# sjz5202/DisenLink

Measured on AMD Instinct MI355X. Metric: edges/sec (aggregate+score) at K=8 d=64, higher is better.
Workload: dtype f32; 1 GPU; squirrel_real (edge list of the parity fixture)(seed 0): N=5201, edge rows=217073, 85/5/10 split, E_sym=342129, scored train pairs P=1009603 (m=5), K=8, d=64, beta=0.5, t=1.0; forward route+aggregate+score_pairs; K=8, d=64, n_nodes=5201, E_sym=342129, P=1009603

## Files before the change

disenlink_amd/csrc/dl_score.hip:

```cpp
#include "dl_fast.h"
#include "dl_score_bwd.h"

namespace dl {
namespace fast {

template <int K, int D, typename T, bool COEF>
__global__ __launch_bounds__(BLOCK, K <= 8 ? 4 : 1) void score_fwd_seg_kernel(dl_csr_plan g, const int32_t* __restrict__ pair_id,
                                                              const int32_t* __restrict__ pair_id2,
                                                              const T* __restrict__ Z, const T* __restrict__ H,
                                                              float t, float* __restrict__ prob,
                                                              float* __restrict__ coef_e,
                                                              float* __restrict__ coef_q) {
    using GE = Geo<K, D, T>;
    constexpr int VEC = GE::VEC, G = GE::G, EPW = GE::EPW, ROW = GE::ROW;
    constexpr int KB = K > 8 ? 8 : K;
    using FLB = FactorLanes<G, KB>;
    constexpr int KBP = FLB::KP;
    __shared__ __attribute__((aligned(16))) float urow[WAVES_PER_BLOCK][2 * ROW];
    const WaveSeg ws = load_wave_seg(g);
    const SegInfo si = ws.si;
    const int wave = ws.wave, lane = lane_id();
    const bool active = ws.active;
    if (active) stage_u_rows<K, D, T>(urow[wave], Z, H, (size_t)si.grow);
    __syncthreads();
    if (!active) return;
    const int c = lane % G, grp = lane / G;
    const int kbb = FLB::factor_base(c);
    int my_col = si.grow, my_pair = 0, my_pair2 = -1;
    if (si.beg + lane < si.end) {
        my_col = g.col[si.beg + lane];
        my_pair = pair_id[si.beg + lane];
        if (pair_id2 != nullptr) my_pair2 = pair_id2[si.beg + lane];
    }
    for (int base = si.beg; base < si.end; base += EPW) {
        const int it = base + grp;
        const bool live = it < si.end;
        const size_t v = (size_t)entry_scalar<EPW>(my_col, base - si.beg, grp);
        const int q = entry_scalar<EPW>(my_pair, base - si.beg, grp);
        const int q2 = entry_scalar<EPW>(my_pair2, base - si.beg, grp);
        float term = 0.0f;
#pragma unroll
        for (int b0 = 0; b0 < K; b0 += KB) {
            float pq[KBP], ps[KBP];
#pragma unroll
            for (int k = 0; k < KBP; ++k) {
                const bool in = k < KB && b0 + k < K;
                const int kk = in ? b0 + k : 0;
                pq[k] = in ? dot(load_f32<VEC>(&urow[wave][ROW + kk * D + c * VEC]), Tab<T>::load(H + v * ROW + kk * D + c * VEC)) : 0.0f;
                ps[k] = in ? dot(load_f32<VEC>(&urow[wave][kk * D + c * VEC]), Tab<T>::load(Z + v * ROW + kk * D + c * VEC)) : 0.0f;
            }
            TransposedReduce<KBP, G / 2>::run(pq, c);
            TransposedReduce<KBP, G / 2>::run(ps, c);
#pragma unroll
            for (int i = 0; i < FLB::VPL; ++i) {
                const int k = b0 + kbb + i;
                if (FLB::primary(c) && kbb + i < KB && k < K) {
                    const float ek = expf(div_t(ps[i], t));
                    const float qe = pq[i] * ek;
                    term += qe;
                    if (COEF && live) {
                        coef_e[(size_t)q * K + k] = ek;
                        coef_q[(size_t)q * K + k] = qe;
                        if (q2 >= 0) {
                            coef_e[(size_t)q2 * K + k] = ek;
                            coef_q[(size_t)q2 * K + k] = qe;
                        }
                    }
                }
            }
        }
        const float logit = group_allreduce_sum<G>(term);
        if (live && c == 0) {
            const float p = sigmoid_ref(logit);
            prob[q] = p;
            if (q2 >= 0) prob[q2] = p;
        }
    }
}

constexpr int FWD_WAVE_MAXW = 6;
template <int K, int D>
struct FwdWave {
    static constexpr bool ok = D == 64 && (K == 4 || K == 8);
    static constexpr int NJ = K * D / 256, U = 4;
};

template <int K, int D, bool T1, bool COEF, bool FOLD>
__global__ __launch_bounds__(BLOCK) __attribute__((amdgpu_waves_per_eu(4, FWD_WAVE_MAXW))) void score_fwd_wave_kernel(dl_csr_plan g, const int32_t* __restrict__ pair_id,
                                                                  const int32_t* __restrict__ pair_id2,
                                                                  const float* __restrict__ Z, const float* __restrict__ H, float t,
                                                                  float* __restrict__ prob, float* __restrict__ coef_e,
                                                                  float* __restrict__ coef_q) {
    using FW = FwdWave<K, D>;
    constexpr int NJ = FW::NJ, U = FW::U, ROW = K * D;
    static_assert(D == 64 && NJ >= 1 && U * NJ <= 8, "one DPP row of 16 lanes per factor slice; at most 8 exponents per row and step");
    __shared__ __attribute__((aligned(16))) float4 urow[WAVES_PER_BLOCK][2 * ROW / 4];
    __shared__ int ent_q[WAVES_PER_BLOCK][(FOLD ? 2 : 1) * DL_WAVE];
    const WaveSeg ws = load_wave_seg(g);
    if (!ws.active) return;
    const SegInfo si = ws.si;
    const int wave = ws.wave, lane = lane_id();
    const int i = lane & 15, r = lane >> 4;
    float4* const mine = urow[wave];
#pragma unroll
    for (int j = 0; j < NJ; ++j) {
        mine[j * 64 + lane] = *reinterpret_cast<const float4*>(Z + (size_t)si.grow * ROW + (j * 64 + lane) * 4);
        mine[ROW / 4 + j * 64 + lane] = *reinterpret_cast<const float4*>(H + (size_t)si.grow * ROW + (j * 64 + lane) * 4);
    }
    int my_col = si.grow, my_q = 0, my_q2 = -1;
    if (si.beg + lane < si.end) {
        my_col = g.col[si.beg + lane];
        my_q = pair_id[si.beg + lane];
        if constexpr (FOLD) my_q2 = pair_id2[si.beg + lane];
    }
    ent_q[wave][lane] = my_q;
    if constexpr (FOLD) ent_q[wave][DL_WAVE + lane] = my_q2;
    const int len = si.end - si.beg;
    auto do_step = [&](const int step, auto tail, const int n_live) {
        constexpr bool TAIL = decltype(tail)::value;
        float4 zv[U][NJ], hv[U][NJ];
#pragma unroll
        for (int e = 0; e < U; ++e) {
            if (!TAIL || e < n_live) {
                const size_t v = (size_t)(unsigned)__builtin_amdgcn_readlane(my_col, (step * U + e) & 63);
                const auto* zr = uniform_row<dl_vf4>(Z, v * ROW * sizeof(float));
                const auto* hr = uniform_row<dl_vf4>(H, v * ROW * sizeof(float));
#pragma unroll
                for (int j = 0; j < NJ; ++j) {
                    zv[e][j] = as_float4(zr[(unsigned)(lane + j * 64)]);
                    hv[e][j] = as_float4(hr[(unsigned)(lane + j * 64)]);
                }
            } else {
#pragma unroll
                for (int j = 0; j < NJ; ++j) zv[e][j] = hv[e][j] = make_float4(0.0f, 0.0f, 0.0f, 0.0f);
            }
        }
        float val[16];
#pragma unroll
        for (int x = 0; x < 16; ++x) val[x] = 0.0f;
#pragma unroll
        for (int j = 0; j < NJ; ++j) {
            const float4 a4 = mine[j * 64 + lane], b4 = mine[ROW / 4 + j * 64 + lane];
#pragma unroll
            for (int e = 0; e < U; ++e) {
                val[j * 4 + e] = dot4_packed(a4, zv[e][j]);
                val[8 + j * 4 + e] = dot4_packed(b4, hv[e][j]);
            }
            __builtin_amdgcn_sched_barrier(0);
        }
        TransposedReduce<16, 8>::run(val, i);
        const float mine_v = val[0];
        const float ex = expf(T1 ? mine_v : mine_v / t);
        const float ttv = mine_v * xor_lane<8>(ex);
        float term = ttv;
        if constexpr (NJ == 2) term += xor_lane<4>(ttv);
        const float logit = add_xor<32>(add_xor<16>(term));
        const float p = sigmoid_ref(logit);
        const int idx = step * U + (i & 3);
        const bool live = idx < len;
        const int qq = ent_q[wave][idx & 63];
        int qq2 = -1;
        if constexpr (FOLD) qq2 = ent_q[wave][DL_WAVE + (idx & 63)];
        if (lane >= 8 && lane < 12 && live) {
            prob[qq] = p;
            if (FOLD && qq2 >= 0) prob[qq2] = p;
        }
        if constexpr (COEF) {
            const int k = 4 * ((i & 7) >> 2) + r;
            if (live && (NJ == 2 || (i & 7) < 4)) {
                if (i < 8) coef_e[(size_t)qq * K + k] = ex;
                else coef_q[(size_t)qq * K + k] = ttv;
                if (FOLD && qq2 >= 0) {
                    if (i < 8) coef_e[(size_t)qq2 * K + k] = ex;
                    else coef_q[(size_t)qq2 * K + k] = ttv;
                }
            }
        }
    };
    const int nfull = len / U;
    for (int step = 0; step < nfull; ++step) do_step(step, std::false_type{}, U);
    if (len % U != 0) do_step(nfull, std::true_type{}, len % U);
}

namespace hub {
constexpr int WAVES = 8, THREADS = WAVES * DL_WAVE;

typedef int dl_vi4 __attribute__((ext_vector_type(4)));
__device__ __forceinline__ dl_vi4 plan_words(const int32_t* a, int idx) {
    const auto* g = (const __attribute__((address_space(1))) int32_t*)a;
    return reinterpret_cast<const __attribute__((address_space(4))) dl_vi4*>((const __attribute__((address_space(4))) int32_t*)g)[idx];
}

struct StepWords {
    dl_vi4 v, u, q, p;
};

template <int K, int D, bool T1, bool COEF, bool FOLD>
__global__ __launch_bounds__(THREADS) __attribute__((amdgpu_waves_per_eu(4, 4))) void score_fwd_wave_kernel(
    dl_pair_hub h, const float* __restrict__ Z, const float* __restrict__ H, float t, float* __restrict__ prob,
    float* __restrict__ coef_e, float* __restrict__ coef_q) {
    using FW = FwdWave<K, D>;
    constexpr int NJ = FW::NJ, U = FW::U, ROW = K * D, R4 = 2 * ROW / 4;
    static_assert(D == 64 && NJ >= 1 && U == 4 && U * NJ <= 8, "the step geometry of score_fwd_wave_kernel");
    static_assert(DL_HUB_W == 2 * WAVES, "every wave stages two rows of the block");
    __shared__ __attribute__((aligned(16))) float4 urow[DL_HUB_W * R4];
    const int x = blockIdx.x % h.n_slices;
    const int it = h.slice_item0[x] + (int)(blockIdx.x / h.n_slices);
    if (it >= h.slice_item0[x + 1]) return;
    const int wave = wave_index(), lane = lane_id();
    const int i = lane & 15, r = lane >> 4;
    const int blk = h.item_block[it];
    const int s_a = h.item_step[4 * it], s_b = h.item_step[4 * it + 1], s_c = h.item_step[4 * it + 2],
              s_end = h.item_step[4 * it + 3];
#pragma unroll
    for (int rr = 0; rr < 2; ++rr) {
        const int ul = 2 * wave + rr;
        const int row = h.block_row[blk * DL_HUB_W + ul];
#pragma unroll
        for (int j = 0; j < NJ; ++j) {
            float4 a = make_float4(0.0f, 0.0f, 0.0f, 0.0f), b = a;
            if (row >= 0) {
                a = *reinterpret_cast<const float4*>(Z + (size_t)row * ROW + (j * 64 + lane) * 4);
                b = *reinterpret_cast<const float4*>(H + (size_t)row * ROW + (j * 64 + lane) * 4);
            }
            urow[ul * R4 + j * 64 + lane] = a;
            urow[ul * R4 + ROW / 4 + j * 64 + lane] = b;
        }
    }
    __syncthreads();
    auto fetch = [&](const int step) {
        const int s = __builtin_amdgcn_readfirstlane(step);
        StepWords w;
        w.v = plan_words(h.step_v, s), w.u = plan_words(h.step_u, s), w.q = plan_words(h.step_q, s);
        w.p = dl_vi4{-1, -1, -1, -1};
        if constexpr (FOLD) w.p = plan_words(h.step_q2, s);
        return w;
    };
    auto do_step = [&](const StepWords& w, auto shape, auto last) {
        constexpr int NV = decltype(shape)::value;
        constexpr bool LAST = decltype(last)::value;
        const int sv[4] = {w.v.x, w.v.y, w.v.z, w.v.w}, su[4] = {w.u.x, w.u.y, w.u.z, w.u.w}, sq[4] = {w.q.x, w.q.y, w.q.z, w.q.w},
                  sq2[4] = {w.p.x, w.p.y, w.p.z, w.p.w};
        float4 zv[NV][NJ], hv[NV][NJ];
#pragma unroll
        for (int n = 0; n < NV; ++n) {
            if (!LAST || sv[n] >= 0) {
                const size_t v = (size_t)(unsigned)sv[n];
                const auto* zr = uniform_row<dl_vf4>(Z, v * ROW * sizeof(float));
                const auto* hr = uniform_row<dl_vf4>(H, v * ROW * sizeof(float));
#pragma unroll
                for (int j = 0; j < NJ; ++j) {
                    zv[n][j] = as_float4(zr[(unsigned)(lane + j * 64)]);
                    hv[n][j] = as_float4(hr[(unsigned)(lane + j * 64)]);
                }
            } else {
#pragma unroll
                for (int j = 0; j < NJ; ++j) zv[n][j] = hv[n][j] = make_float4(0.0f, 0.0f, 0.0f, 0.0f);
            }
        }
        float val[16];
#pragma unroll
        for (int q = 0; q < 16; ++q) val[q] = 0.0f;
#pragma unroll
        for (int j = 0; j < NJ; ++j) {
            float4 a4[U], b4[U];
#pragma unroll
            for (int e = 0; e < U; ++e) {
                const float4* mine = urow + (su[e] & (DL_HUB_W - 1)) * R4;
                a4[e] = mine[j * 64 + lane], b4[e] = mine[ROW / 4 + j * 64 + lane];
            }
            __builtin_amdgcn_sched_barrier(0);
#pragma unroll
            for (int e = 0; e < U; ++e) {
                val[j * 4 + e] = dot4_packed(a4[e], zv[e * NV / 4][j]);
                val[8 + j * 4 + e] = dot4_packed(b4[e], hv[e * NV / 4][j]);
            }
            __builtin_amdgcn_sched_barrier(0);
        }
        TransposedReduce<16, 8>::run(val, i);
        const float mine_v = val[0];
        const float ex = expf(T1 ? mine_v : mine_v / t);
        const float ttv = mine_v * xor_lane<8>(ex);
        float term = ttv;
        if constexpr (NJ == 2) term += xor_lane<4>(ttv);
        const float logit = add_xor<32>(add_xor<16>(term));
        const float p = sigmoid_ref(logit);
        const int e_me = i & 3;
        const int qq = e_me == 0 ? sq[0] : e_me == 1 ? sq[1] : e_me == 2 ? sq[2] : sq[3];
        const int qq2 = e_me == 0 ? sq2[0] : e_me == 1 ? sq2[1] : e_me == 2 ? sq2[2] : sq2[3];
        const bool live = qq >= 0;
        if (lane >= 8 && lane < 12 && live) {
            prob[qq] = p;
            if (FOLD && qq2 >= 0) prob[qq2] = p;
        }
        if constexpr (COEF) {
            const int k = 4 * ((i & 7) >> 2) + r;
            if (live && (NJ == 2 || (i & 7) < 4)) {
                if (i < 8) coef_e[(size_t)qq * K + k] = ex;
                else coef_q[(size_t)qq * K + k] = ttv;
                if (FOLD && qq2 >= 0) {
                    if (i < 8) coef_e[(size_t)qq2 * K + k] = ex;
                    else coef_q[(size_t)qq2 * K + k] = ttv;
                }
            }
        }
    };
    using FULL = std::false_type;
    using LAST = std::true_type;
    constexpr std::integral_constant<int, 4> SHAPE_A{};
    constexpr std::integral_constant<int, 2> SHAPE_B{};
    constexpr std::integral_constant<int, 1> SHAPE_C{};
    int s = s_a + wave;
    StepWords nxt = {};
    if (s < s_end) nxt = fetch(s);
    auto take = [&](const int step) {
        const StepWords w = nxt;
        if (step + WAVES < s_end) nxt = fetch(step + WAVES);
        return w;
    };
    for (; s < s_b - 1; s += WAVES) do_step(take(s), SHAPE_A, FULL{});
    if (s == s_b - 1) do_step(take(s), SHAPE_A, LAST{}), s += WAVES;
    for (; s < s_c - 1; s += WAVES) do_step(take(s), SHAPE_B, FULL{});
    if (s == s_c - 1) do_step(take(s), SHAPE_B, LAST{}), s += WAVES;
    for (; s < s_end; s += WAVES) do_step(take(s), SHAPE_C, FULL{});
}
}

template <int K, int D, typename T>
__global__ __launch_bounds__(BLOCK) void score_allpairs_kernel(const T* __restrict__ Z, const T* __restrict__ H, int N,
                                                               float t, int n_slices, int slice_w, int chunks_per_u,
                                                               float* __restrict__ prob) {
    using GE = Geo<K, D, T>;
    constexpr int VEC = GE::VEC, G = GE::G, EPW = GE::EPW, ROW = GE::ROW;
    constexpr int KB = K > 8 ? 8 : K;
    using FLB = FactorLanes<G, KB>;
    constexpr int KBP = FLB::KP;
    constexpr int VCH = 256;
    __shared__ __attribute__((aligned(16))) float urow[WAVES_PER_BLOCK][2 * ROW];
    const int wave = threadIdx.x >> 6, lane = lane_id();
    const int x = blockIdx.x % n_slices;
    const int item = (blockIdx.x / n_slices) * WAVES_PER_BLOCK + wave;
    const int u = item / chunks_per_u, ch = item - u * chunks_per_u;
    const int v0 = x * slice_w + ch * VCH;
    const int v1 = min(min(v0 + VCH, (x + 1) * slice_w), N);
    const bool active = u < N && v0 < v1;
    if (active) stage_u_rows<K, D, T>(urow[wave], Z, H, (size_t)u);
    __syncthreads();
    if (!active) return;
    const int c = lane % G, grp = lane / G;
    const int kbb = FLB::factor_base(c);
    for (int base = v0; base < v1; base += EPW) {
        const int vi = base + grp;
        const bool live = vi < v1;
        const size_t v = (size_t)(live ? vi : v0);
        float term = 0.0f;
#pragma unroll
        for (int b0 = 0; b0 < K; b0 += KB) {
            float pq[KBP], ps[KBP];
#pragma unroll
            for (int k = 0; k < KBP; ++k) {
                const bool in = k < KB && b0 + k < K;
                const int kk = in ? b0 + k : 0;
                pq[k] = in ? dot(load_f32<VEC>(&urow[wave][ROW + kk * D + c * VEC]), Tab<T>::load(H + v * ROW + kk * D + c * VEC)) : 0.0f;
                ps[k] = in ? dot(load_f32<VEC>(&urow[wave][kk * D + c * VEC]), Tab<T>::load(Z + v * ROW + kk * D + c * VEC)) : 0.0f;
            }
            TransposedReduce<KBP, G / 2>::run(pq, c);
            TransposedReduce<KBP, G / 2>::run(ps, c);
#pragma unroll
            for (int i = 0; i < FLB::VPL; ++i)
                if (FLB::primary(c) && kbb + i < KB && b0 + kbb + i < K) term += pq[i] * expf(div_t(ps[i], t));
        }
        const float logit = group_allreduce_sum<G>(term);
        if (live && c == 0) prob[(size_t)u * N + vi] = sigmoid_ref(logit);
    }
}

template <int K, int D, typename T, int PASS>
__global__ __launch_bounds__(BLOCK) void score_bwd_coef_seg_kernel(dl_csr_plan g, const int32_t* __restrict__ inc_pair,
                                                                   const T* __restrict__ X, float t,
                                                                   const float* __restrict__ prob,
                                                                   const float* __restrict__ g_prob,
                                                                   const float* __restrict__ coef,
                                                                   float* __restrict__ out, float* __restrict__ part) {
    using GE = Geo<K, D, T>;
    constexpr int VEC = GE::VEC, G = GE::G, EPW = GE::EPW, ROW = GE::ROW;
    using US = Stage<K, D, T, 1>;
    __shared__ __attribute__((aligned(16))) float red[US::FLOATS];
    const WaveSeg ws = load_wave_seg(g);
    const SegInfo si = ws.si;
    const int lane = lane_id();
    const int c = lane % G, grp = lane / G;
    if (ws.active) {
        Chunk<VEC> acc[K];
#pragma unroll
        for (int k = 0; k < K; ++k) acc[k] = zero_chunk<VEC>();
        int my_col = si.grow, my_pair = 0;
        float my_gl = 0.0f;
        if (si.beg + lane < si.end) {
            my_col = g.col[si.beg + lane];
            my_pair = inc_pair[si.beg + lane];
            const float pr = prob[my_pair];
            my_gl = g_prob[my_pair] * pr * (1.0f - pr);
            if (PASS == 0) my_gl = div_t(my_gl, t);
        }
        for (int base = si.beg; base < si.end; base += EPW) {
            const int idx = base + grp - si.beg;
            const size_t v = (size_t)__shfl(my_col, idx, DL_WAVE);
            const int q = __shfl(my_pair, idx, DL_WAVE);
            const float gl = __shfl(my_gl, idx, DL_WAVE);
            float ck[K];
            if constexpr (K % 4 == 0) {
#pragma unroll
                for (int k = 0; k < K; k += 4) {
                    const float4 t4 = *reinterpret_cast<const float4*>(coef + (size_t)q * K + k);
                    ck[k] = t4.x; ck[k + 1] = t4.y; ck[k + 2] = t4.z; ck[k + 3] = t4.w;
                }
            } else {
#pragma unroll
                for (int k = 0; k < K; ++k) ck[k] = coef[(size_t)q * K + k];
            }
#pragma unroll
            for (int b0 = 0; b0 < K; b0 += 8) {
                Chunk<VEC> xv[8];
#pragma unroll
                for (int k = 0; k < 8; ++k)
                    if (b0 + k < K) xv[k] = Tab<T>::load(X + v * ROW + (b0 + k) * D + c * VEC);
#pragma unroll
                for (int k = 0; k < 8; ++k)
                    if (b0 + k < K) fma_chunk(acc[b0 + k], gl * ck[b0 + k], xv[k]);
            }
        }
        US::put(red, ws.wave, grp, c, acc, 0);
    }
    __syncthreads();
    if (!ws.head) return;
    float4 r[US::NQ];
    US::sum(red, ws.wave, ws.n_unit, lane, r);
    float* o = si.slot < 0 ? out + (size_t)si.grow * ROW : part + (size_t)si.slot * ROW;
#pragma unroll
    for (int q = 0; q < US::NQ; ++q) {
        const int x = q * DL_WAVE + lane;
        if (x < US::F4) store4(o + 4 * x, r[q]);
    }
}

struct AllpairsGeo { int n_slices, slice_w, chunks_per_u; long long items; unsigned blocks; };
static AllpairsGeo allpairs_geo(int N, size_t row_bytes) {
    AllpairsGeo g;
    const double table = 2.0 * N * (double)row_bytes;
    g.n_slices = table <= 8.0 * 8.0 * (4 << 20) && N >= 64 ? 8 : 1;
    g.slice_w = (N + g.n_slices - 1) / g.n_slices;
    g.chunks_per_u = (g.slice_w + 255) / 256;
    g.items = (long long)N * g.chunks_per_u;
    g.blocks = (unsigned)(g.n_slices * ((g.items + WAVES_PER_BLOCK - 1) / WAVES_PER_BLOCK));
    return g;
}

template <int K, int D, typename T>
struct ScoreOps {
    static constexpr int ROW = K * D;
    static int score_fwd(const dl_pair_incidence* by_u, const void* Z, const void* H, float t, float* prob,
                         float* coef, hipStream_t st) {
        const dl_csr_plan* g = &by_u->csr;
        float* coef_q = coef ? coef + (size_t)by_u->n_pairs * K : nullptr;
        if constexpr (std::is_same<T, float>::value && FwdWave<K, D>::ok) {
            if (g->seg_len <= 64 && g->seg_len % FwdWave<K, D>::U == 0 && !config().fwd_group_kernel) {
                auto pick = [&](auto launch) {
                    auto fold = [&](auto t1, auto cf) {
                        if (by_u->inc_pair2) launch(t1, cf, std::true_type{});
                        else launch(t1, cf, std::false_type{});
                    };
                    if (coef) { if (t == 1.0f) fold(std::true_type{}, std::true_type{}); else fold(std::false_type{}, std::true_type{}); }
                    else { if (t == 1.0f) fold(std::true_type{}, std::false_type{}); else fold(std::false_type{}, std::false_type{}); }
                };
                auto wave_plan = [&](const dl_csr_plan* c, const int32_t* pair, const int32_t* pair2) {
                    pick([&](auto t1, auto cf, auto fo) {
                        hipLaunchKernelGGL((score_fwd_wave_kernel<K, D, decltype(t1)::value, decltype(cf)::value, decltype(fo)::value>),
                                           dim3(seg_blocks(c)), dim3(BLOCK), 0, st, *c, pair, pair2, (const float*)Z,
                                           (const float*)H, t, prob, coef, coef_q);
                    });
                };
                const dl_pair_hub* hp = config().fwd_hub ? by_u->hub : nullptr;
                if (hp != nullptr && hp->n_items > 0) {
                    pick([&](auto t1, auto cf, auto fo) {
                        hipLaunchKernelGGL((hub::score_fwd_wave_kernel<K, D, decltype(t1)::value, decltype(cf)::value, decltype(fo)::value>),
                                           dim3((unsigned)hp->n_slices * (unsigned)hp->slice_max_item), dim3(hub::THREADS), 0,
                                           st, *hp, (const float*)Z, (const float*)H, t, prob, coef, coef_q);
                    });
                    if (hp->rest.n_entries > 0) wave_plan(&hp->rest, hp->rest_pair, hp->rest_pair2);
                    return check_launch("score_pairs_fwd(fast, hub blocks + wave per entry)");
                }
                wave_plan(g, by_u->inc_pair, by_u->inc_pair2);
                return check_launch("score_pairs_fwd(fast, wave per entry)");
            }
        }
        if (coef)
            hipLaunchKernelGGL((score_fwd_seg_kernel<K, D, T, true>), dim3(seg_blocks(g)), dim3(BLOCK), 0, st, *g,
                               by_u->inc_pair, by_u->inc_pair2, (const T*)Z, (const T*)H, t, prob, coef, coef_q);
        else
            hipLaunchKernelGGL((score_fwd_seg_kernel<K, D, T, false>), dim3(seg_blocks(g)), dim3(BLOCK), 0, st, *g,
                               by_u->inc_pair, by_u->inc_pair2, (const T*)Z, (const T*)H, t, prob, coef, coef_q);
        return check_launch("score_pairs_fwd(fast)");
    }

    static int score_allpairs(const void* Z, const void* H, int N, float t, float* prob, hipStream_t st) {
        const AllpairsGeo g = allpairs_geo(N, ROW * sizeof(T));
        hipLaunchKernelGGL((score_allpairs_kernel<K, D, T>), dim3(g.blocks), dim3(BLOCK), 0, st, (const T*)Z, (const T*)H, N,
                           t, g.n_slices, g.slice_w, g.chunks_per_u, prob);
        return check_launch("score_allpairs_fwd(fast)");
    }

    static int score_bwd(const dl_pair_incidence* inc, const void* Z, const void* H, float t, const float* prob,
                         const float* g_prob, const float* coef, float* dZ, float* dH, float* part, hipStream_t st) {
        const dl_csr_plan* g = &inc->csr;
        const float* no_x = nullptr;
        if (coef) {
            const float* coef_q = coef + (size_t)inc->n_pairs * K;
            float* part_h = part + (size_t)g->n_slots * ROW;
            hipLaunchKernelGGL((score_bwd_coef_seg_kernel<K, D, T, 0>), dim3(seg_blocks(g)), dim3(BLOCK), 0, st, *g,
                               inc->inc_pair, (const T*)Z, t, prob, g_prob, coef_q, dZ, part);
            hipLaunchKernelGGL((score_bwd_coef_seg_kernel<K, D, T, 1>), dim3(seg_blocks(g)), dim3(BLOCK), 0, st, *g,
                               inc->inc_pair, (const T*)H, t, prob, g_prob, coef, dH, part_h);
            if (g->n_multi > 0)
                hipLaunchKernelGGL((row_combine_kernel<ROW, float, float>), dim3(g->n_multi, 2), dim3(BLOCK), 0, st, *g,
                                   part, ROW, no_x, 0.0f, 1.0f, dZ, 0, part_h, dH);
            return check_launch("score_pairs_bwd(fast, stored terms)");
        }
        hipLaunchKernelGGL((score_bwd_seg_kernel<K, D, T, false>), dim3(seg_blocks(g)), dim3(BLOCK), 0, st, *g, inc->inc_pair,
                           (const T*)Z, (const T*)H, t, prob, g_prob, dZ, dH, part);
        if (g->n_multi > 0)
            hipLaunchKernelGGL((row_combine_kernel<ROW, float, float>), dim3(g->n_multi, 2), dim3(BLOCK), 0, st, *g, part,
                               2 * ROW, no_x, 0.0f, 1.0f, dZ, 0, part + ROW, dH);
        return check_launch("score_pairs_bwd(fast)");
    }
};

}

int fast_score_pairs_fwd(const dl_pair_incidence* by_u, const void* Z, const void* H, int K, int d, int dtype,
                         float t, float* prob, float* coef, hipStream_t st) {
#define X_F32(KK, DD) if (K == KK && d == DD) return fast::ScoreOps<KK, DD, float>::score_fwd(by_u, Z, H, t, prob, coef, st);
#define X_BF16(KK, DD) if (K == KK && d == DD) return fast::ScoreOps<KK, DD, fast::bf16_t>::score_fwd(by_u, Z, H, t, prob, coef, st);
    DL_DISPATCH(X)
#undef X_F32
#undef X_BF16
}

int fast_score_pairs_bwd(const dl_pair_incidence* inc, const void* Z, const void* H, int K, int d, int dtype,
                         float t, const float* prob, const float* g_prob, const float* coef, float* dZ, float* dH,
                         float* part, hipStream_t st) {
#define X_F32(KK, DD) if (K == KK && d == DD) return fast::ScoreOps<KK, DD, float>::score_bwd(inc, Z, H, t, prob, g_prob, coef, dZ, dH, part, st);
#define X_BF16(KK, DD) if (K == KK && d == DD) return fast::ScoreOps<KK, DD, fast::bf16_t>::score_bwd(inc, Z, H, t, prob, g_prob, coef, dZ, dH, part, st);
    DL_DISPATCH(X)
#undef X_F32
#undef X_BF16
}

int fast_score_allpairs_fwd(const void* Z, const void* H, int N, int K, int d, int dtype, float t, float* prob,
                            hipStream_t st) {
#define X_F32(KK, DD) if (K == KK && d == DD) return fast::ScoreOps<KK, DD, float>::score_allpairs(Z, H, N, t, prob, st);
#define X_BF16(KK, DD) if (K == KK && d == DD) return fast::ScoreOps<KK, DD, fast::bf16_t>::score_allpairs(Z, H, N, t, prob, st);
    DL_DISPATCH(X)
#undef X_F32
#undef X_BF16
}

void fast_score_allpairs_form(int N, int K, int d, int dtype, int* out) {
    const fast::AllpairsGeo g = fast::allpairs_geo(N, (size_t)K * d * (dtype == DL_BF16 ? sizeof(fast::bf16_t) : sizeof(float)));
    out[1] = (int)g.items;
    out[2] = (int)g.blocks;
    out[3] = g.n_slices;
    out[4] = g.slice_w;
    out[5] = g.chunks_per_u;
}

}
```

Baseline: 8.341 billion edges/s.

## Batch pair logits across steps and use masked DPP transposed reduction

In the score wave kernel without coefficient output, each wave now collects one logit per step into a per-lane slot over 16 steps. Every 16 steps it runs sigmoid once and each of the 64 lanes writes its own probability, replacing the per-step sigmoid and 4-lane scattered store. Pair-index loads move into a per-batch gather instead of per-step scalar plan loads. The 16-wide transposed reduction is replaced with inline DPP asm using bank masks to cut instructions. The cost is more complex lane bookkeeping and hand-written asm hazards (s_nop) that could be fragile.

```diff
diff --git a/disenlink_amd/csrc/dl_score.hip b/disenlink_amd/csrc/dl_score.hip
--- a/disenlink_amd/csrc/dl_score.hip
+++ b/disenlink_amd/csrc/dl_score.hip
@@ -195,6 +195,45 @@
     dl_vi4 v, u, q, p;
 };
 
+__device__ __forceinline__ void transposed_reduce16_masked(float* v, int c) {
+    float a[8], b[4];
+    asm volatile("s_nop 1\n\t"
+                 "v_add_f32_dpp %0, %8, %8 row_ror:8 row_mask:0xf bank_mask:0x3\n\t"
+                 "v_add_f32_dpp %1, %9, %9 row_ror:8 row_mask:0xf bank_mask:0x3\n\t"
+                 "v_add_f32_dpp %2, %10, %10 row_ror:8 row_mask:0xf bank_mask:0x3\n\t"
+                 "v_add_f32_dpp %3, %11, %11 row_ror:8 row_mask:0xf bank_mask:0x3\n\t"
+                 "v_add_f32_dpp %4, %12, %12 row_ror:8 row_mask:0xf bank_mask:0x3\n\t"
+                 "v_add_f32_dpp %5, %13, %13 row_ror:8 row_mask:0xf bank_mask:0x3\n\t"
+                 "v_add_f32_dpp %6, %14, %14 row_ror:8 row_mask:0xf bank_mask:0x3\n\t"
+                 "v_add_f32_dpp %7, %15, %15 row_ror:8 row_mask:0xf bank_mask:0x3\n\t"
+                 "v_add_f32_dpp %0, %16, %16 row_ror:8 row_mask:0xf bank_mask:0xc\n\t"
+                 "v_add_f32_dpp %1, %17, %17 row_ror:8 row_mask:0xf bank_mask:0xc\n\t"
+                 "v_add_f32_dpp %2, %18, %18 row_ror:8 row_mask:0xf bank_mask:0xc\n\t"
+                 "v_add_f32_dpp %3, %19, %19 row_ror:8 row_mask:0xf bank_mask:0xc\n\t"
+                 "v_add_f32_dpp %4, %20, %20 row_ror:8 row_mask:0xf bank_mask:0xc\n\t"
+                 "v_add_f32_dpp %5, %21, %21 row_ror:8 row_mask:0xf bank_mask:0xc\n\t"
+                 "v_add_f32_dpp %6, %22, %22 row_ror:8 row_mask:0xf bank_mask:0xc\n\t"
+                 "v_add_f32_dpp %7, %23, %23 row_ror:8 row_mask:0xf bank_mask:0xc"
+                 : "=&v"(a[0]), "=&v"(a[1]), "=&v"(a[2]), "=&v"(a[3]), "=&v"(a[4]), "=&v"(a[5]), "=&v"(a[6]), "=&v"(a[7])
+                 : "v"(v[0]), "v"(v[1]), "v"(v[2]), "v"(v[3]), "v"(v[4]), "v"(v[5]), "v"(v[6]), "v"(v[7]), "v"(v[8]), "v"(v[9]),
+                   "v"(v[10]), "v"(v[11]), "v"(v[12]), "v"(v[13]), "v"(v[14]), "v"(v[15]));
+    asm volatile("s_nop 1\n\t"
+                 "v_add_f32_dpp %0, %4, %4 row_shl:4 row_mask:0xf bank_mask:0x5\n\t"
+                 "v_add_f32_dpp %1, %5, %5 row_shl:4 row_mask:0xf bank_mask:0x5\n\t"
+                 "v_add_f32_dpp %2, %6, %6 row_shl:4 row_mask:0xf bank_mask:0x5\n\t"
+                 "v_add_f32_dpp %3, %7, %7 row_shl:4 row_mask:0xf bank_mask:0x5\n\t"
+                 "v_add_f32_dpp %0, %8, %8 row_shr:4 row_mask:0xf bank_mask:0xa\n\t"
+                 "v_add_f32_dpp %1, %9, %9 row_shr:4 row_mask:0xf bank_mask:0xa\n\t"
+                 "v_add_f32_dpp %2, %10, %10 row_shr:4 row_mask:0xf bank_mask:0xa\n\t"
+                 "v_add_f32_dpp %3, %11, %11 row_shr:4 row_mask:0xf bank_mask:0xa\n\t"
+                 "s_nop 1"
+                 : "=&v"(b[0]), "=&v"(b[1]), "=&v"(b[2]), "=&v"(b[3])
+                 : "v"(a[0]), "v"(a[1]), "v"(a[2]), "v"(a[3]), "v"(a[4]), "v"(a[5]), "v"(a[6]), "v"(a[7]));
+#pragma unroll
+    for (int q = 0; q < 4; ++q) v[q] = b[q];
+    TransposedReduce<4, 2>::run(v, c);
+}
+
 template <int K, int D, bool T1, bool COEF, bool FOLD>
 __global__ __launch_bounds__(THREADS) __attribute__((amdgpu_waves_per_eu(4, 4))) void score_fwd_wave_kernel(
     dl_pair_hub h, const float* __restrict__ Z, const float* __restrict__ H, float t, float* __restrict__ prob,
@@ -203,6 +242,7 @@
     constexpr int NJ = FW::NJ, U = FW::U, ROW = K * D, R4 = 2 * ROW / 4;
     static_assert(D == 64 && NJ >= 1 && U == 4 && U * NJ <= 8, "the step geometry of score_fwd_wave_kernel");
     static_assert(DL_HUB_W == 2 * WAVES, "every wave stages two rows of the block");
+    constexpr bool BATCH = !COEF;
     __shared__ __attribute__((aligned(16))) float4 urow[DL_HUB_W * R4];
     const int x = blockIdx.x % h.n_slices;
     const int it = h.slice_item0[x] + (int)(blockIdx.x / h.n_slices);
@@ -231,10 +271,38 @@
     auto fetch = [&](const int step) {
         const int s = __builtin_amdgcn_readfirstlane(step);
         StepWords w;
-        w.v = plan_words(h.step_v, s), w.u = plan_words(h.step_u, s), w.q = plan_words(h.step_q, s);
-        w.p = dl_vi4{-1, -1, -1, -1};
-        if constexpr (FOLD) w.p = plan_words(h.step_q2, s);
+        w.v = plan_words(h.step_v, s), w.u = plan_words(h.step_u, s);
+        w.q = w.p = dl_vi4{-1, -1, -1, -1};
+        if constexpr (!BATCH) {
+            w.q = plan_words(h.step_q, s);
+            if constexpr (FOLD) w.p = plan_words(h.step_q2, s);
+        }
         return w;
+    };
+    const int slot_step = lane >> 2;
+    float lg = 0.0f;
+    int nb = 0, pq = -1, pq2 = -1;
+    auto open = [&](const int s0) {
+        const int sb = s0 + WAVES * slot_step;
+        pq = pq2 = -1;
+        if (sb < s_end) {
+            pq = h.step_q[4 * sb + (lane & 3)];
+            if constexpr (FOLD) pq2 = h.step_q2[4 * sb + (lane & 3)];
+        }
+    };
+    auto flush = [&]() {
+        const float p = sigmoid_ref(lg);
+        if (pq >= 0) prob[pq] = p;
+        if (FOLD && pq2 >= 0) prob[pq2] = p;
+    };
+    auto tick = [&](const int step) {
+        if constexpr (BATCH) {
+            if (__builtin_expect(nb == 16, 0)) {
+                flush();
+                nb = 0;
+                open(step + WAVES);
+            }
+        }
     };
     auto do_step = [&](const StepWords& w, auto shape, auto last) {
         constexpr int NV = decltype(shape)::value;
@@ -277,30 +345,39 @@
             }
             __builtin_amdgcn_sched_barrier(0);
         }
-        TransposedReduce<16, 8>::run(val, i);
+        transposed_reduce16_masked(val, i);
         const float mine_v = val[0];
         const float ex = expf(T1 ? mine_v : mine_v / t);
         const float ttv = mine_v * xor_lane<8>(ex);
         float term = ttv;
         if constexpr (NJ == 2) term += xor_lane<4>(ttv);
-        const float logit = add_xor<32>(add_xor<16>(term));
-        const float p = sigmoid_ref(logit);
-        const int e_me = i & 3;
-        const int qq = e_me == 0 ? sq[0] : e_me == 1 ? sq[1] : e_me == 2 ? sq[2] : sq[3];
-        const int qq2 = e_me == 0 ? sq2[0] : e_me == 1 ? sq2[1] : e_me == 2 ? sq2[2] : sq2[3];
-        const bool live = qq >= 0;
-        if (lane >= 8 && lane < 12 && live) {
-            prob[qq] = p;
-            if (FOLD && qq2 >= 0) prob[qq2] = p;
-        }
-        if constexpr (COEF) {
-            const int k = 4 * ((i & 7) >> 2) + r;
-            if (live && (NJ == 2 || (i & 7) < 4)) {
-                if (i < 8) coef_e[(size_t)qq * K + k] = ex;
-                else coef_q[(size_t)qq * K + k] = ttv;
-                if (FOLD && qq2 >= 0) {
-                    if (i < 8) coef_e[(size_t)qq2 * K + k] = ex;
-                    else coef_q[(size_t)qq2 * K + k] = ttv;
+        if constexpr (BATCH) {
+            int tb = __float_as_int(term);
+            tb = __builtin_amdgcn_update_dpp(tb, tb, 0x114, 0xF, 0x8, false);
+            tb = __builtin_amdgcn_update_dpp(tb, tb, 0x128, 0xF, 0x3, false);
+            const float logit = add_xor<32>(add_xor<16>(__int_as_float(tb)));
+            lg = slot_step == nb ? logit : lg;
+            ++nb;
+        } else {
+            const float logit = add_xor<32>(add_xor<16>(term));
+            const float p = sigmoid_ref(logit);
+            const int e_me = i & 3;
+            const int qq = e_me == 0 ? sq[0] : e_me == 1 ? sq[1] : e_me == 2 ? sq[2] : sq[3];
+            const int qq2 = e_me == 0 ? sq2[0] : e_me == 1 ? sq2[1] : e_me == 2 ? sq2[2] : sq2[3];
+            const bool live = qq >= 0;
+            if (lane >= 8 && lane < 12 && live) {
+                prob[qq] = p;
+                if (FOLD && qq2 >= 0) prob[qq2] = p;
+            }
+            if constexpr (COEF) {
+                const int k = 4 * ((i & 7) >> 2) + r;
+                if (live && (NJ == 2 || (i & 7) < 4)) {
+                    if (i < 8) coef_e[(size_t)qq * K + k] = ex;
+                    else coef_q[(size_t)qq * K + k] = ttv;
+                    if (FOLD && qq2 >= 0) {
+                        if (i < 8) coef_e[(size_t)qq2 * K + k] = ex;
+                        else coef_q[(size_t)qq2 * K + k] = ttv;
+                    }
                 }
             }
         }
@@ -318,11 +395,15 @@
         if (step + WAVES < s_end) nxt = fetch(step + WAVES);
         return w;
     };
-    for (; s < s_b - 1; s += WAVES) do_step(take(s), SHAPE_A, FULL{});
-    if (s == s_b - 1) do_step(take(s), SHAPE_A, LAST{}), s += WAVES;
-    for (; s < s_c - 1; s += WAVES) do_step(take(s), SHAPE_B, FULL{});
-    if (s == s_c - 1) do_step(take(s), SHAPE_B, LAST{}), s += WAVES;
-    for (; s < s_end; s += WAVES) do_step(take(s), SHAPE_C, FULL{});
+    if constexpr (BATCH) open(s);
+    for (; s < s_b - 1; s += WAVES) do_step(take(s), SHAPE_A, FULL{}), tick(s);
+    if (s == s_b - 1) do_step(take(s), SHAPE_A, LAST{}), tick(s), s += WAVES;
+    for (; s < s_c - 1; s += WAVES) do_step(take(s), SHAPE_B, FULL{}), tick(s);
+    if (s == s_c - 1) do_step(take(s), SHAPE_B, LAST{}), tick(s), s += WAVES;
+    for (; s < s_end; s += WAVES) do_step(take(s), SHAPE_C, FULL{}), tick(s);
+    if constexpr (BATCH) {
+        if (nb > 0) flush();
+    }
 }
 }
 
```

Result: faster. 8.723 billion edges/s (median of 6 runs) (+4.6%).
